# williamyang98/FM-Radio

Measured on AMD Instinct MI355X. Metric: IQ MSamples/sec demodulated to stereo+RDS per GPU; channels @ real-time, higher is better.
Workload: dtype f32 (tolerance mode: FIR operands split into 2 x bf16 on the matrix cores, 3 products per tap, fp32 accumulate; everything else fp32)

## Files before the change

### fm-radio_amd/capi.py

```python
from __future__ import annotations

import ctypes as C
import re
import subprocess
from pathlib import Path
from typing import NamedTuple

import numpy as np

PKG_DIR = Path(__file__).resolve().parent
ROOT = PKG_DIR.parent
CSRC = PKG_DIR / "csrc"
HEADER = ROOT / "include" / "fmdemod.h"
DEBUG_HEADER = ROOT / "include" / "fmdemod_debug.h"

FMD_AUDIO_LPR, FMD_AUDIO_LMR, FMD_AUDIO_STEREO = 0, 1, 2
FMD_FLAG_KEEP_TAPS = 1
FMD_FLAG_NO_PIPELINE = 2
FMD_FLAG_PLL_TIME_PARALLEL = 4
FMD_FLAG_PLL_LOW_WORK = 8
FMD_FLAG_PLL_K8 = 16
FMD_FLAG_PLL_STREAM_ORDER = 32
FMD_FLAG_FAST_MATH = 64
FMD_FLAG_RDS_DECODE = 128
# ... 325 lines not shown
    L.fmd_get_rds_symbols.argtypes = [H, C.c_void_p, C.c_void_p]
    L.fmd_get_rds_bytes.argtypes = [H, C.c_void_p, C.c_int, C.c_void_p]
    L.fmd_rds_bytes_dev.argtypes = [H, C.POINTER(C.c_void_p), C.POINTER(C.c_void_p), C.POINTER(C.c_int)]
    L.fmd_get_stream.argtypes = [H, C.c_char_p, C.c_void_p, C.c_size_t, C.POINTER(C.c_size_t)]
    L.fmd_selftest_atan2.argtypes = [C.c_void_p, C.c_void_p, C.c_void_p, C.c_size_t]
    L.fmd_selftest_atan2_table.argtypes = [C.c_void_p, C.c_void_p, C.c_void_p, C.c_size_t]
    L.fmd_selftest_atan2_table_u8.argtypes = [C.c_void_p, C.c_void_p, C.c_void_p, C.c_size_t]
    L.fmd_selftest_atan2_small.argtypes = [C.c_void_p, C.c_void_p, C.c_void_p, C.c_void_p, C.c_size_t]
    L.fmd_selftest_fast_math.argtypes = [C.c_int, C.c_void_p, C.c_void_p, C.c_void_p, C.c_size_t]
    L.fmd_get_spec_stats.argtypes = [H, C.c_void_p, C.c_int]
    L.fmd_design_pll_span.argtypes = [C.c_int, C.c_void_p, C.c_void_p, C.c_void_p, C.c_void_p]
    L.fmd_profile_enable.argtypes = [H, C.c_int]
    L.fmd_debug_split_front.argtypes = [H, C.c_int]
    L.fmd_debug_pll_adaptive.argtypes = [H, C.c_int, C.c_int]
    L.fmd_debug_extract_pairing.argtypes = [H, C.c_int]
    L.fmd_debug_plan.argtypes = [C.POINTER(Config), C.c_int, C.c_int, C.c_int, C.POINTER(PlanInfo)]
    L.fmd_debug_block_plan.argtypes = [C.POINTER(Config), C.POINTER(PlanFacts), C.c_int, C.POINTER(BlockPlanInfo)]
    L.fmd_profile_read.argtypes = [H, C.POINTER(KernelTime), C.c_int, C.POINTER(C.c_int)]
    L.fmd_chan_design.argtypes = [C.c_double, C.c_double, C.c_int, C.c_void_p, C.POINTER(C.c_int), C.POINTER(C.c_int)]
    L.fmd_chan_default_taps_per_phase.restype = C.c_int
    L.fmd_chan_default_taps_per_phase.argtypes = [C.c_double, C.c_double]
    L.fmd_chan_create.argtypes = [C.POINTER(ChanConfig), C.POINTER(C.c_void_p)]
    L.fmd_chan_reset.argtypes = [C.c_void_p]
    L.fmd_chan_info.argtypes = [C.c_void_p] + [C.POINTER(C.c_int)] * 4
    L.fmd_chan_get_taps.argtypes = [C.c_void_p, C.c_void_p, C.c_size_t]
    for fmt in ("cf32", "u8", "s8", "s16"):
        getattr(L, f"fmd_chan_process_{fmt}_dev").argtypes = [C.c_void_p, C.c_void_p, C.c_size_t, C.c_void_p, C.c_size_t, C.POINTER(C.c_size_t), C.c_void_p]
    L.fmd_scan_default_nfft.restype = C.c_int
    L.fmd_scan_default_nfft.argtypes = [C.c_double]
    L.fmd_scan_default_params.restype = None
# ... 471 lines not shown
        return rc

    def wait_input(self, stream=None):
        stream = _stream_ptr(stream)
        self._check(self.L.fmd_wait_input(self.h, C.c_void_p(stream)))

    def synchronize(self):
        self._check(self.L.fmd_synchronize(self.h))

    def pll_adaptive(self, k16_max_channels: int, time_parallel_max_channels: int = 7168) -> None:
        self._check(self.L.fmd_debug_pll_adaptive(self.h, int(k16_max_channels), int(time_parallel_max_channels)))

    def set_extract_pairing(self, mode: int) -> None:
        self._check(self.L.fmd_debug_extract_pairing(self.h, int(mode)))

    def set_output_lag(self, on: bool) -> None:
        self._check(self.L.fmd_set_output_lag(self.h, 1 if on else 0))

    def outputs_block(self) -> int:
        b = C.c_long(-1)
        self._check(self.L.fmd_outputs_block(self.h, C.byref(b)))
        return int(b.value)

    def wait_outputs(self, stream=None):
        stream = _stream_ptr(stream)
        self._check(self.L.fmd_wait_outputs(self.h, C.c_void_p(stream)))

    def release_outputs(self, stream=None):
        stream = _stream_ptr(stream)
        self._check(self.L.fmd_release_outputs(self.h, C.c_void_p(stream)))
# ... 1027 lines not shown
```

### fm-radio_amd/csrc/fmd_api.cpp

```cpp
#include <hip/hip_runtime.h>

#include <algorithm>
#include <cstdarg>
#include <cstdio>
#include <cstdlib>
#include <cstring>
#include <map>
#include <new>
#include <string>
#include <vector>

#include "fmd_design.h"
#include "fmd_kernels.h"
#include "fmd_plan.h"
#include "fmd_schedule.h"
#include "fmd_tables.h"
#include "fmdemod.h"
#include "fmdemod_debug.h"

using namespace fmd;

struct ProfiledBlock { hipEvent_t t0[ST_COUNT], t1[ST_COUNT]; bool used[ST_COUNT]; };

struct fmd_handle_s {
    fmd_config cfg{};
    LaunchCtx ctx{};
    fmd_coeffs base{};
    std::vector<fmd_controls> controls;
    bool controls_dirty = true;
    bool deemph_on = false;
    bool deemph_linger = false;
    std::vector<void*> allocs;
    void* d_in = nullptr;
// ... 467 lines not shown
    h->pipelined = (cfg->flags & FMD_FLAG_NO_PIPELINE) == 0;
    if (h->pipelined) warn_hw_queues_once();
    {
        std::vector<hipEvent_t*> evs = {&h->ev_in};
        for (int i = 0; i < kSlots; i++) { evs.push_back(&h->ev_P[i]); evs.push_back(&h->ev_F[i]); evs.push_back(&h->ev_A[i]); evs.push_back(&h->ev_B[i]); evs.push_back(&h->ev_E[i]); evs.push_back(&h->ev_X[i]); evs.push_back(&h->ev_C[i]); evs.push_back(&h->ev_D[i]); }
        for (hipEvent_t* ev : evs) {
            hipError_t e = hipEventCreateWithFlags(ev, hipEventDisableTiming);
            if (e != hipSuccess) return bail(fail(h, FMD_ERR_DEVICE, "event: %s", hipGetErrorString(e)));
        }
    }
    h->ctx.d = dims_of(*cfg, m);
    const Dims& d = h->ctx.d;
    h->ctx.plan = make_plan(d.C, d.m, d.n_fm_out, d.n_est, cfg->flags);
    refresh_block_plan(h->ctx);
    h->ctx.pll_unlocked_now = false; h->ctx.pll_launch_no = 0;
    h->bytes_cap = 16 * (d.n_rds / 256 + 1);
    h->ctx.bytes_cap = h->bytes_cap;
    h->ctx.keep_taps = (cfg->flags & FMD_FLAG_KEEP_TAPS) ? 1 : 0;
    h->ctx.rds_decode = (cfg->flags & FMD_FLAG_RDS_DECODE) ? 1 : 0;
    h->ctx.fast = (cfg->flags & FMD_FLAG_FAST_MATH) ? 1 : 0;

    fmd_controls def;
    fmd_default_controls(&def);
    h->controls.assign((size_t)d.C, def);
    design_all(&h->base, cfg->fs_baseband, &def);
    fill_ctx_coeffs(h);

    Buffers& b = h->ctx.b;
    const size_t C = (size_t)d.C;
    int rc = FMD_OK;
// ... 624 lines not shown
    *out = fmd_block_plan_info{b.iq_streams, (int)b.front, (int)in.front_input, in.front_tile, b.front_warmup, in.front_workgroups, b.front_lds_pad,
                               (int)in.predecim, in.predecim_tile, in.predecim_workgroups, b.deemph_pilot_sums, b.deemph_workgroups, p.power_rows,
                               (int)b.lmr_phase, b.extract_tile, b.extract_bp, b.extract_nt, b.extract_pair, b.extract_grid_x, (int)b.rds, b.rds_partials};
    return FMD_OK;
}

int fmd_debug_extract_pairing(fmd_handle h, int mode) {
    if (!h || mode < 0 || mode > 2) return FMD_ERR_ARG;
    int rc = fmd_synchronize(h);
    if (rc) return rc;
    h->ctx.facts.extract_pairing = mode;
    refresh_block_plan(h->ctx);
    return FMD_OK;
}

int fmd_profile_enable(fmd_handle h, int on) {
    if (!h) return FMD_ERR_ARG;
    h->sched.set_profiling(on < 0 ? 0 : (on > 3 ? 3 : on));
    return FMD_OK;
}

int fmd_profile_read(fmd_handle h, fmd_kernel_time* out, int cap, int* n_out) {
    if (!h || !out || !n_out || cap <= 0) return FMD_ERR_ARG;
    int rc = fmd_synchronize(h);
    if (rc) return rc;
    int n = 0;
    for (ProfiledBlock* pm : h->marks) {
        for (int i = 0; i < ST_COUNT; i++) {
            if (!pm->used[i]) continue;
            float ms = 0.0f;
// ... 187 lines not shown
```

### fm-radio_amd/csrc/fmd_kernels.h

```cpp
#pragma once

#include <hip/hip_runtime.h>
#include <stdint.h>
#include <cstdlib>

#include "fmd_plan.h"
#include "fmd_schedule.h"
#include "fmd_tables.h"
#include "fmdemod.h"

namespace fmd {

#ifdef FMD_DEV_HOOKS
inline const char* dev_env(const char* name) { return std::getenv(name); }
#else
inline const char* dev_env(const char*) { return nullptr; }
#endif

struct FrontTaps {
    float b_fm_in[64];
    float b_fm_out[64];
    float b_hilbert_odd[32];
    float fm_gain;
};
// ... 125 lines not shown
    Dims d;
    Buffers b;
    FrontTaps front;
    RdsTaps rds_taps;
    LoopCoeffs loops;
    int keep_taps;
    int fast;
    int bytes_cap;
    int rds_decode;
    RdsDecBufs rds_dec;
    Plan plan;
    PlanFacts facts;
    BlockPlan block;
    Dims d_front;
    unsigned pll_launch_no;
    bool pll_unlocked_now;
};

inline void refresh_block_plan(LaunchCtx& ctx) {
    ctx.block = make_block_plan(ctx.plan, ctx.facts);
    ctx.d_front = ctx.d;
    if (ctx.d.m > 1) { ctx.d_front.N = ctx.d.n_fm_in; ctx.d_front.m = 1; }
}

inline TapPtrs tap_ptrs(const LaunchCtx& ctx, int buf) {
    TapPtrs t{};
    float* p = ctx.b.taps[buf];
    if (!p) return t;
    const size_t nf = (size_t)ctx.d.C * ctx.d.n_fm_out, nr = (size_t)ctx.d.C * ctx.d.n_rds;
    t.pilot = reinterpret_cast<float2*>(p); p += 2 * nf;
// ... 31 lines not shown
```

### fm-radio_amd/csrc/fmd_kernels.hip

```cpp
#include "fmd_kernels.h"
#include <hip/hip_ext.h>
#include <cstdlib>
#include <type_traits>
#include "fmd_math.h"

#define FMD_LAUNCH(r, first, last, kern, grid, block, lds, s, ...)                                                   \
    do {                                                                                                             \
        hipEvent_t e0_ = (first) ? (r).t0 : nullptr, e1_ = (last) ? ((r).t1 ? (r).t1 : (r).done) : nullptr;         \
        if (e0_ || e1_) hipExtLaunchKernelGGL(kern, grid, block, lds, s, e0_, e1_, 0, __VA_ARGS__);                  \
        else hipLaunchKernelGGL(kern, grid, block, lds, s, __VA_ARGS__);                                             \
    } while (0)


namespace fmd {

static constexpr int kWave = 64;

__device__ __forceinline__ float& st(float* state, int field, int C, int c) { return state[(size_t)field * C + c]; }

#include "fmd_kernels_sparse.inc"

static constexpr int kDeemphWarmup = 128;
template <int TT = 512>
struct FrontGeom {
// ... 364 lines not shown
        }
    }
}

template <typename InT, int TT, int WU, bool FUSED = false>
__global__ __launch_bounds__(256, FUSED ? 6 : 5) void k_front_mfma(Dims d, const InT* __restrict__ in, const float2* __restrict__ tail_in,
                                                    float2* __restrict__ tail_out, float* __restrict__ fo_pl, float fm_gain,
                                                    const float* __restrict__ deemph, const uint4* __restrict__ tab, float4* __restrict__ pv_pl,
                                                    const PllSparseTab* __restrict__ sp, PllFusedArgs pf) {
    using G = FrontGeomM<TT, WU>;
    constexpr int T = G::T, NW = G::NW;
    extern __shared__ __attribute__((aligned(16))) float smem[];
    int bid = (int)blockIdx.x;
    if constexpr (FUSED) {
        if (bid < pf.n_wg) {
            pll_sparse_body(d, bid * 4 + (int)(threadIdx.x >> 6), (int)(threadIdx.x & (kWave - 1)), pf.pv, pf.hist_in, pf.hist_out, pf.fo, pf.fo_next, pf.poly, pf.poly_next,
                            pf.state, pf.k, pf.tab, 0, pf.spec_stats);
            return;
        }
        bid -= pf.n_wg;
    }
    float* theta = smem + G::OFF_THETA;

    const int tiles = d.n_fm_out / T;
    const int c = bid / tiles, tile = bid % tiles, o0 = tile * T, tid = threadIdx.x;
    __builtin_assume(tid >= 0 && tid < 256);
    const int lane = tid & (kWave - 1), lq = lane >> 4;
    const int g_lo = 2 * o0 - G::TAIL;
    const InT* in_c = in + (size_t)c * d.N;
    const float2* tail_c = tail_in + (size_t)c * d.tail_base + (d.tail_base - G::TAIL);

    FrontOps op;
// ... 327 lines not shown
    static constexpr int MINWG = (U8 && M == 4) ? 5 : 4;
    static_assert(NCOLS % NSUB == 0 && NBS % 8 == 0 && SEG * (CS - 1) + 32 * KS <= NBS && GF::NWB >= NPH + 1, "geometry");
};
template <int M, typename InT, bool FUSED>
__global__ __launch_bounds__(256, (FUSED ? FrontPreGeom<M, sizeof(InT) == 2>::MINWG : 4)) void k_front_pre_mfma(Dims d, const InT* __restrict__ in, const float2* __restrict__ pre_tail_in, float2* __restrict__ pre_tail_out,
                                                           const float2* __restrict__ tail_in, float2* __restrict__ tail_out, float* __restrict__ fo_pl, float fm_gain,
                                                           const uint4* __restrict__ tab_pre, const uint4* __restrict__ tab, float4* __restrict__ pv_pl,
                                                           const PllSparseTab* __restrict__ sp, PllFusedArgs pf) {
    constexpr bool U8 = sizeof(InT) == 2;
    using G = FrontPreGeom<M, U8>;
    constexpr int NBS = G::NBS, KS = G::KS, SEG = G::SEG, NH = G::NH, NWD = G::NWD, CS = G::CS;
    extern __shared__ __attribute__((aligned(16))) float smem[];
    int bid = (int)blockIdx.x;
    if constexpr (FUSED) {
        if (bid < pf.n_wg) {
            pll_sparse_body(d, bid * 4 + (int)(threadIdx.x >> 6), (int)(threadIdx.x & (kWave - 1)), pf.pv, pf.hist_in, pf.hist_out, pf.fo, pf.fo_next, pf.poly, pf.poly_next,
                            pf.state, pf.k, pf.tab, 0, pf.spec_stats);
            return;
        }
        bid -= pf.n_wg;
    }
    uint32_t* arr = reinterpret_cast<uint32_t*>(smem);
    float* region = smem + G::ARR_WORDS;
    const int tiles = d.n_fm_out / 1024;
    const int c = bid / tiles, tile = bid % tiles, o0 = tile * 1024, tid = threadIdx.x;
    __builtin_assume(tid >= 0 && tid < 256);
    const int lane = tid & (kWave - 1), wv = tid >> 6, lrow = lane & 15, lq = lane >> 4;
    const int g_first = M * (2 * o0 - 64) + M - 64 - G::SH;
    const InT* in_c = in + (size_t)c * d.N;
    const float2* ptail_c = pre_tail_in + (size_t)c * G::HIST;
    auto word_of = [](int pair) { return pair + 4 * (pair / (SEG / 2)); };

// ... 1709 lines not shown

__global__ void k_reset(Dims d, float* __restrict__ state) {
    const int c = blockIdx.x * blockDim.x + threadIdx.x;
    if (c >= d.C) return;
    for (int f = 0; f < S_NUM_FIELDS; f++) st(state, f, d.C, c) = 0.0f;
    st(state, S_AGC_PILOT_GAIN, d.C, c) = 0.1f;
    st(state, S_AGC_RDS_GAIN, d.C, c) = 0.1f;
}

template <int... Vs, typename F>
static bool with_constant(int v, F&& f) { return ((v == Vs ? (f(std::integral_constant<int, Vs>{}), true) : false) || ...); }
static hipError_t launched(bool found) { return found ? hipGetLastError() : hipErrorInvalidConfiguration; }

static_assert(kDeemphWarmup == kFrontDeemphWarmup && PredecimGeom<4>::TP == 512 && PredecimGeom<8>::TP == 512, "fmd_plan.cpp's geometry");

static PllFusedArgs fused_pilot_args(const LaunchCtx& ctx, const SlotRef* pll) {
    const Buffers& b = ctx.b;
    if (!pll) { PllFusedArgs none{}; none.state = b.state; return none; }
    const int nxt = (pll->buf + 1) % kSlots;
    return PllFusedArgs{(ctx.d.C + 31) / 32, b.pv_pl[pll->buf], b.pv_hist[pll->par], b.pv_hist[pll->par ^ 1], b.fo_pl[pll->buf], b.fo_pl[nxt],
                        b.pll_poly[pll->buf], b.pll_poly[nxt], b.state, ctx.loops, b.sparse_tab, b.spec_stats};
}

template <typename InT, typename F>
static bool with_front_tile(int tile, F&& f) {
    if constexpr (sizeof(InT) == 4) return with_constant<512, 1024>(tile, f);
    else return with_constant<512, 1024, 2048>(tile, f);
}

template <typename InT>
static hipError_t launch_front(const LaunchCtx& ctx, const BlockPlan::Input& in, SlotRef r, const InT* d_iq, hipStream_t s, const SlotRef* pll) {
    const BlockPlan& bp = ctx.block;
    const Buffers& b = ctx.b;
    const Dims& d = ctx.d_front;
    if (bp.front == FrontKernel::FrontMfma) {
        const PllFusedArgs pf = fused_pilot_args(ctx, pll);
        return launched(with_front_tile<InT>(in.front_tile, [&](auto tt) { with_constant<0, kDeemphWarmup>(bp.front_warmup, [&](auto wu) { with_constant<0, 1>(pll != nullptr, [&](auto fused) {
            constexpr int TT = decltype(tt)::value, WU = decltype(wu)::value;
            using G = FrontGeomM<TT, WU>;
            FMD_LAUNCH(r, true, true, (k_front_mfma<InT, TT, WU, decltype(fused)::value != 0>), dim3((unsigned)(in.front_workgroups + pf.n_wg)), dim3(256),
                       sizeof(float) * G::LDS_FLOATS + bp.front_lds_pad, s, d, d_iq, b.base_tail[r.par], b.base_tail[r.par ^ 1], b.fo_pl[r.buf], ctx.front.fm_gain,
                       b.deemph, b.front_mfma, b.pv_pl[r.buf], b.sparse_tab, pf);
        }); }); }));
    }
    return launched(with_front_tile<InT>(in.front_tile, [&](auto tt) {
        constexpr int TT = decltype(tt)::value;
        FMD_LAUNCH(r, true, true, (k_front<InT, TT>), dim3((unsigned)in.front_workgroups), dim3(256), sizeof(float) * FrontGeom<TT>::LDS_FLOATS, s, d, d_iq, b.base_tail[r.par],
                   b.base_tail[r.par ^ 1], b.fm_out_iq[r.buf], b.fm_out[r.buf], b.fo_tail[r.par ^ 1], ctx.front, ctx.facts.any_deemph ? 1 : 0);
    }));
}

template <int M, typename InT>
static void launch_front_pre(const LaunchCtx& ctx, const BlockPlan::Input& in, SlotRef r, const InT* d_iq, hipStream_t s, const SlotRef* pll) {
    using G = FrontPreGeom<M, sizeof(InT) == 2>;
    const Buffers& b = ctx.b;
    const PllFusedArgs pf = fused_pilot_args(ctx, pll);
    with_constant<0, 1>(pll != nullptr, [&](auto fused) {
        FMD_LAUNCH(r, true, true, (k_front_pre_mfma<M, InT, decltype(fused)::value != 0>), dim3((unsigned)(in.front_workgroups + pf.n_wg)), dim3(256), sizeof(float) * G::LDS_WORDS, s, ctx.d, d_iq,
                   b.pre_tail[r.par], b.pre_tail[r.par ^ 1], b.base_tail[r.par], b.base_tail[r.par ^ 1], b.fo_pl[r.buf], ctx.front.fm_gain, b.front_mfma + kFrontImgU4, b.front_mfma,
                   b.pv_pl[r.buf], b.sparse_tab, pf);
    });
}

template <int M, typename InT>
static void launch_predecim(const LaunchCtx& ctx, const BlockPlan::Input& in, SlotRef r, const InT* d_iq, hipStream_t s) {
    const Buffers& b = ctx.b;
    const dim3 grid((unsigned)in.predecim_workgroups);
    if (in.predecim == PredecimKernel::Mfma) {
        with_constant<256, (sizeof(InT) == 2 ? 8192 : 2048) / M>(in.predecim_tile, [&](auto tp) {
            FMD_LAUNCH(r, true, true, (k_predecim_mfma<M, InT, decltype(tp)::value>), grid, dim3(256), 0, s, ctx.d, d_iq, b.pre_tail[r.par], b.pre_tail[r.par ^ 1],
                       reinterpret_cast<float*>(b.fm_in[r.buf]), b.front_mfma + kFrontImgU4);
// ... 48 lines not shown
}

hipError_t launch_stage_power(const LaunchCtx& ctx, SlotRef r, hipStream_t s) {
    const Dims& d = ctx.d;
    return launched(with_constant<0, 1>(ctx.plan.power_rows, [&](auto rows) {
        FMD_LAUNCH(r, true, true, k_pilot_power<decltype(rows)::value != 0>, dim3(serial_waves(d)), dim3(kWave), 0, s, d, ctx.b.fm_out_iq[r.buf], ctx.b.pilot[r.buf], ctx.b.state,
                   ctx.loops, (int)S_PILOT_POWER0 + r.buf);
    }));
}

hipError_t launch_stage_pll(const LaunchCtx& ctx, SlotRef r, hipStream_t s) {
    const Dims& d = ctx.d;
    if (ctx.fast) {
        const int nxt = (r.buf + 1) % kSlots;
        const bool iq = ctx.block.iq_streams;
        FMD_LAUNCH(r, true, !iq && !r.warm, k_pll_sparse, dim3((unsigned)((d.C + 31) / 32)), dim3(4 * kWave), 0, s, d, ctx.b.pv_pl[r.buf], ctx.b.pv_hist[r.par], ctx.b.pv_hist[r.par ^ 1],
                   ctx.b.fo_pl[r.buf], ctx.b.fo_pl[nxt], ctx.b.pll_poly[r.buf], ctx.b.pll_poly[nxt], ctx.b.state, ctx.loops, ctx.b.sparse_tab, r.warm, ctx.b.spec_stats);
        if (r.warm)
            FMD_LAUNCH(r, false, !iq, k_pll_span, dim3((unsigned)((d.C + 3) / 4)), dim3(kWave), 0, s, d, ctx.b.fo_pl[r.buf], ctx.b.fo_pl[nxt],
                       ctx.b.pll_poly[r.buf], ctx.b.pll_poly[nxt], (float*)nullptr, ctx.b.state, ctx.loops, ctx.b.pilot_tab, ctx.b.span_tab, ctx.b.spec_stats, r.warm == 2 ? 1 : 0);
        if (iq) FMD_LAUNCH(r, false, false, k_poly_to_dt, dim3((unsigned)((size_t)d.n_fm_out * d.C / 256)), dim3(256), 0, s, d, ctx.b.pll_poly[r.buf], ctx.b.pll_dt[r.buf]);
        if (iq) FMD_LAUNCH(r, false, true, k_planes_to_iq, dim3((unsigned)(d.n_fm_out / 256 * d.C)), dim3(256), 0, s, d, ctx.b.fo_pl[r.buf], ctx.b.fm_out_iq[r.buf], ctx.front);
        return hipGetLastError();
    }
    if (ctx.b.taps[r.buf]) hipLaunchKernelGGL(k_pll_taps, dim3((unsigned)((d.C + kWave - 1) / kWave)), dim3(kWave), 0, s, d, ctx.b.pilot[r.buf], ctx.b.state, ctx.loops,
                                              (int)S_PILOT_POWER0 + r.buf, tap_ptrs(ctx, r.buf));
    const PllKernel kernel = pll_kernel(ctx.plan, ctx.pll_unlocked_now);
    if (kernel == PllKernel::LowWork) {
        FMD_LAUNCH(r, true, true, k_pilot_pll_pairs, dim3((unsigned)((d.C + kPllCh - 1) / kPllCh)), dim3(2 * kWave), 0, s, d, ctx.b.pilot[r.buf], ctx.b.pll_dt[r.buf],
                   ctx.b.state, ctx.loops, (int)S_PILOT_POWER0 + r.buf, ctx.b.spec_stats, ctx.b.pll_hint, ctx.pll_launch_no);
        return hipGetLastError();
    }
// ... 134 lines not shown
```

### fm-radio_amd/csrc/fmd_kernels_sparse.inc

```
static constexpr int kRowShr1 = 0x111, kRowShr2 = 0x112, kRowShr4 = 0x114, kRowShr8 = 0x118;
static constexpr int kWaveShr1 = 0x138, kRowBcast15 = 0x142;
template <int CTRL>
__device__ __forceinline__ float dpp_f(float old, float v, bool bound_zero) {
    return bound_zero ? __int_as_float(__builtin_amdgcn_update_dpp(0, __float_as_int(v), CTRL, 0xf, 0xf, true))
                      : __int_as_float(__builtin_amdgcn_update_dpp(__float_as_int(old), __float_as_int(v), CTRL, 0xf, 0xf, false));
}

struct __attribute__((packed, aligned(4))) F4U { float x, y, z, w; };
template <int CTRL, int BANK = 0xf>
__device__ __forceinline__ float dpp0(float v) {
    return __int_as_float(__builtin_amdgcn_update_dpp(0, __float_as_int(v), CTRL, 0xf, BANK, true));
}
__device__ __forceinline__ float sum8_all(float v) {
    v += dpp0<0xB1>(v);
    v += dpp0<0x4E>(v);
    v += dpp0<0x141>(v);
    return v;
}
__device__ __forceinline__ float bcast_lane7_of_8(float v) {
    const int q = __builtin_amdgcn_update_dpp(0, __float_as_int(v), 0xFF, 0xf, 0xf, true);
    return __int_as_float(__builtin_amdgcn_update_dpp(q, q, 0x104, 0xf, 0x5, false));
}
__device__ __forceinline__ float bcast_lane0_of_8(float v) {
    const int q = __builtin_amdgcn_update_dpp(0, __float_as_int(v), 0x00, 0xf, 0xf, true);
// ... 150 lines not shown
        }
    }
    if (spec_stats) {
        if (lane == 0) atomicAdd(&spec_stats[0], (unsigned long long)chunks);
        if (live && mine && kp == 0) { atomicAdd(&spec_stats[3], (unsigned long long)chunks); atomicAdd(&spec_stats[4], (unsigned long long)n); }
        if (lane == 0 && wave_id == 0) { atomicAdd(&spec_stats[6], __builtin_readcyclecounter() - clk0); atomicAdd(&spec_stats[7], __builtin_amdgcn_s_memrealtime() - rt0); }
    }
    if (live && kp < 4) hist_out[(size_t)cs * 4 + kp] = pvr[ncol - 4 + kp];
    if (live) {
        const float4* src = reinterpret_cast<const float4*>(fo + (size_t)cs * fo_stride + n);
        float4* dst = reinterpret_cast<float4*>(fo_next + (size_t)cs * fo_stride);
        for (int i = kp; i < kFoPad / 4; i += KP) dst[i] = src[i];
    }
}

__global__ __launch_bounds__(4 * kWave) void k_pll_sparse(Dims d, const float4* __restrict__ pv, const float4* __restrict__ hist_in, float4* __restrict__ hist_out,
                                                      const float* __restrict__ fo, float* __restrict__ fo_next,
                                                      float4* __restrict__ poly, float4* __restrict__ poly_next,
                                                      float* __restrict__ state, LoopCoeffs k, const PllSparseTab* __restrict__ tab, int warm_block,
                                                      unsigned long long* __restrict__ spec_stats) {
    pll_sparse_body(d, (int)(blockIdx.x * 4 + (threadIdx.x >> 6)), (int)(threadIdx.x & (kWave - 1)), pv, hist_in, hist_out, fo, fo_next, poly, poly_next, state, k, tab,
                    warm_block, spec_stats);
}

struct PllFusedArgs {
    int n_wg;
    const float4* pv; const float4* hist_in; float4* hist_out; const float* fo; float* fo_next; float4* poly; float4* poly_next; float* state; LoopCoeffs k; const PllSparseTab* tab; unsigned long long* spec_stats;
};

__global__ __launch_bounds__(256) void k_pilot_sums(Dims d, const float* __restrict__ fo_pl, float4* __restrict__ pv_pl, const PllSparseTab* __restrict__ sp) {
    const int n = d.n_fm_out, ncol = n / kSparseDec, blocks_per = (ncol + 63) / 64;
    const int c = blockIdx.x / blocks_per, cc = (blockIdx.x % blocks_per) * 64 + (threadIdx.x >> 2), part = threadIdx.x & 3;
    if (cc >= ncol) return;
    const float* x = fo_pl + (size_t)c * (kFoPad + n) + kFoPad + kSparseDec * cc;
    const float* w = ((part & 1) ? sp->wim : sp->wre) + ((part < 2) ? kSparseDec : 0);
    float a0_ = 0.0f, a1_ = 0.0f;
#pragma unroll
    for (int i = 0; i < kSparseDec; i += 2) { a0_ = fmaf(w[i], x[i], a0_); a1_ = fmaf(w[i + 1], x[i + 1], a1_); }
    reinterpret_cast<float*>(pv_pl + (size_t)c * ncol + cc)[part] = a0_ + a1_;
}

__global__ __launch_bounds__(256) void k_poly_to_dt(Dims d, const float4* __restrict__ poly, float* __restrict__ pll_dt) {
    const int n = d.n_fm_out, spans = n / kSpan;
// ... 9 lines not shown
```

Before: 275,000.

## Add rider PLL body packing 16 stations per wave for fused pilot stage

Adds a new sparse-PLL body in which each wave handles S stations instead of 8. Lanes compute span-phase points grouped eight per station and hand them through LDS to per-station loop-update lanes. The fused front-kernel pilot stage uses this body by default whenever enough LDS is available and the indices fit in 32 bits, which cuts the number of pilot workgroups. A debug switch selects the old body or the standalone rider kernel. The trade is extra LDS traffic and serialized per-chunk loop updates per lane in exchange for better lane utilization.

```diff
diff --git a/fm-radio_amd/capi.py b/fm-radio_amd/capi.py
--- a/fm-radio_amd/capi.py
+++ b/fm-radio_amd/capi.py
@@ -363,6 +363,7 @@
     L.fmd_debug_split_front.argtypes = [H, C.c_int]
     L.fmd_debug_pll_adaptive.argtypes = [H, C.c_int, C.c_int]
     L.fmd_debug_extract_pairing.argtypes = [H, C.c_int]
+    L.fmd_debug_pilot_body.argtypes = [H, C.c_int]
     L.fmd_debug_plan.argtypes = [C.POINTER(Config), C.c_int, C.c_int, C.c_int, C.POINTER(PlanInfo)]
     L.fmd_debug_block_plan.argtypes = [C.POINTER(Config), C.POINTER(PlanFacts), C.c_int, C.POINTER(BlockPlanInfo)]
     L.fmd_profile_read.argtypes = [H, C.POINTER(KernelTime), C.c_int, C.POINTER(C.c_int)]
@@ -864,6 +865,9 @@
     def set_extract_pairing(self, mode: int) -> None:
         self._check(self.L.fmd_debug_extract_pairing(self.h, int(mode)))
 
+    def set_pilot_body(self, mode: int) -> None:
+        self._check(self.L.fmd_debug_pilot_body(self.h, int(mode)))
+
     def set_output_lag(self, on: bool) -> None:
         self._check(self.L.fmd_set_output_lag(self.h, 1 if on else 0))
 
diff --git a/fm-radio_amd/csrc/fmd_api.cpp b/fm-radio_amd/csrc/fmd_api.cpp
--- a/fm-radio_amd/csrc/fmd_api.cpp
+++ b/fm-radio_amd/csrc/fmd_api.cpp
@@ -17,6 +17,7 @@
 #include "fmd_tables.h"
 #include "fmdemod.h"
 #include "fmdemod_debug.h"
+#include "fmdemod_pilot_debug.h"
 
 using namespace fmd;
 
@@ -514,6 +515,7 @@
     h->ctx.plan = make_plan(d.C, d.m, d.n_fm_out, d.n_est, cfg->flags);
     refresh_block_plan(h->ctx);
     h->ctx.pll_unlocked_now = false; h->ctx.pll_launch_no = 0;
+    h->ctx.pilot_body = 0;
     h->bytes_cap = 16 * (d.n_rds / 256 + 1);
     h->ctx.bytes_cap = h->bytes_cap;
     h->ctx.keep_taps = (cfg->flags & FMD_FLAG_KEEP_TAPS) ? 1 : 0;
@@ -1168,6 +1170,14 @@
     return FMD_OK;
 }
 
+int fmd_debug_pilot_body(fmd_handle h, int mode) {
+    if (!h || mode < 0 || mode > 2) return FMD_ERR_ARG;
+    int rc = fmd_synchronize(h);
+    if (rc) return rc;
+    h->ctx.pilot_body = mode;
+    return FMD_OK;
+}
+
 int fmd_profile_enable(fmd_handle h, int on) {
     if (!h) return FMD_ERR_ARG;
     h->sched.set_profiling(on < 0 ? 0 : (on > 3 ? 3 : on));
diff --git a/fm-radio_amd/csrc/fmd_kernels.h b/fm-radio_amd/csrc/fmd_kernels.h
--- a/fm-radio_amd/csrc/fmd_kernels.h
+++ b/fm-radio_amd/csrc/fmd_kernels.h
@@ -163,6 +163,7 @@
     BlockPlan block;
     Dims d_front;
     unsigned pll_launch_no;
+    int pilot_body;
     bool pll_unlocked_now;
 };
 
diff --git a/fm-radio_amd/csrc/fmd_kernels.hip b/fm-radio_amd/csrc/fmd_kernels.hip
--- a/fm-radio_amd/csrc/fmd_kernels.hip
+++ b/fm-radio_amd/csrc/fmd_kernels.hip
@@ -402,8 +402,7 @@
     int bid = (int)blockIdx.x;
     if constexpr (FUSED) {
         if (bid < pf.n_wg) {
-            pll_sparse_body(d, bid * 4 + (int)(threadIdx.x >> 6), (int)(threadIdx.x & (kWave - 1)), pf.pv, pf.hist_in, pf.hist_out, pf.fo, pf.fo_next, pf.poly, pf.poly_next,
-                            pf.state, pf.k, pf.tab, 0, pf.spec_stats);
+            fused_pilot_stage(d, bid, pf, smem);
             return;
         }
         bid -= pf.n_wg;
@@ -761,8 +760,7 @@
     int bid = (int)blockIdx.x;
     if constexpr (FUSED) {
         if (bid < pf.n_wg) {
-            pll_sparse_body(d, bid * 4 + (int)(threadIdx.x >> 6), (int)(threadIdx.x & (kWave - 1)), pf.pv, pf.hist_in, pf.hist_out, pf.fo, pf.fo_next, pf.poly, pf.poly_next,
-                            pf.state, pf.k, pf.tab, 0, pf.spec_stats);
+            fused_pilot_stage(d, bid, pf, smem);
             return;
         }
         bid -= pf.n_wg;
@@ -2502,11 +2500,13 @@
 
 static_assert(kDeemphWarmup == kFrontDeemphWarmup && PredecimGeom<4>::TP == 512 && PredecimGeom<8>::TP == 512, "fmd_plan.cpp's geometry");
 
-static PllFusedArgs fused_pilot_args(const LaunchCtx& ctx, const SlotRef* pll) {
+static PllFusedArgs fused_pilot_args(const LaunchCtx& ctx, const SlotRef* pll, size_t lds_bytes) {
     const Buffers& b = ctx.b;
     if (!pll) { PllFusedArgs none{}; none.state = b.state; return none; }
     const int nxt = (pll->buf + 1) % kSlots;
-    return PllFusedArgs{(ctx.d.C + 31) / 32, b.pv_pl[pll->buf], b.pv_hist[pll->par], b.pv_hist[pll->par ^ 1], b.fo_pl[pll->buf], b.fo_pl[nxt],
+    const bool rider = ctx.pilot_body != 1 && lds_bytes >= sizeof(float) * kRiderLdsFloats && rider_indexable(ctx.d);
+    const int per_wg = rider ? 4 * kRiderS : 32;
+    return PllFusedArgs{(ctx.d.C + per_wg - 1) / per_wg, rider ? 1 : 0, b.pv_pl[pll->buf], b.pv_hist[pll->par], b.pv_hist[pll->par ^ 1], b.fo_pl[pll->buf], b.fo_pl[nxt],
                         b.pll_poly[pll->buf], b.pll_poly[nxt], b.state, ctx.loops, b.sparse_tab, b.spec_stats};
 }
 
@@ -2522,10 +2522,10 @@
     const Buffers& b = ctx.b;
     const Dims& d = ctx.d_front;
     if (bp.front == FrontKernel::FrontMfma) {
-        const PllFusedArgs pf = fused_pilot_args(ctx, pll);
         return launched(with_front_tile<InT>(in.front_tile, [&](auto tt) { with_constant<0, kDeemphWarmup>(bp.front_warmup, [&](auto wu) { with_constant<0, 1>(pll != nullptr, [&](auto fused) {
             constexpr int TT = decltype(tt)::value, WU = decltype(wu)::value;
             using G = FrontGeomM<TT, WU>;
+            const PllFusedArgs pf = fused_pilot_args(ctx, pll, sizeof(float) * G::LDS_FLOATS + bp.front_lds_pad);
             FMD_LAUNCH(r, true, true, (k_front_mfma<InT, TT, WU, decltype(fused)::value != 0>), dim3((unsigned)(in.front_workgroups + pf.n_wg)), dim3(256),
                        sizeof(float) * G::LDS_FLOATS + bp.front_lds_pad, s, d, d_iq, b.base_tail[r.par], b.base_tail[r.par ^ 1], b.fo_pl[r.buf], ctx.front.fm_gain,
                        b.deemph, b.front_mfma, b.pv_pl[r.buf], b.sparse_tab, pf);
@@ -2542,7 +2542,7 @@
 static void launch_front_pre(const LaunchCtx& ctx, const BlockPlan::Input& in, SlotRef r, const InT* d_iq, hipStream_t s, const SlotRef* pll) {
     using G = FrontPreGeom<M, sizeof(InT) == 2>;
     const Buffers& b = ctx.b;
-    const PllFusedArgs pf = fused_pilot_args(ctx, pll);
+    const PllFusedArgs pf = fused_pilot_args(ctx, pll, sizeof(float) * G::LDS_WORDS);
     with_constant<0, 1>(pll != nullptr, [&](auto fused) {
         FMD_LAUNCH(r, true, true, (k_front_pre_mfma<M, InT, decltype(fused)::value != 0>), dim3((unsigned)(in.front_workgroups + pf.n_wg)), dim3(256), sizeof(float) * G::LDS_WORDS, s, ctx.d, d_iq,
                    b.pre_tail[r.par], b.pre_tail[r.par ^ 1], b.base_tail[r.par], b.base_tail[r.par ^ 1], b.fo_pl[r.buf], ctx.front.fm_gain, b.front_mfma + kFrontImgU4, b.front_mfma,
@@ -2621,8 +2621,12 @@
     if (ctx.fast) {
         const int nxt = (r.buf + 1) % kSlots;
         const bool iq = ctx.block.iq_streams;
-        FMD_LAUNCH(r, true, !iq && !r.warm, k_pll_sparse, dim3((unsigned)((d.C + 31) / 32)), dim3(4 * kWave), 0, s, d, ctx.b.pv_pl[r.buf], ctx.b.pv_hist[r.par], ctx.b.pv_hist[r.par ^ 1],
-                   ctx.b.fo_pl[r.buf], ctx.b.fo_pl[nxt], ctx.b.pll_poly[r.buf], ctx.b.pll_poly[nxt], ctx.b.state, ctx.loops, ctx.b.sparse_tab, r.warm, ctx.b.spec_stats);
+        if (ctx.pilot_body == 2 && rider_indexable(d))
+            FMD_LAUNCH(r, true, !iq && !r.warm, k_pll_sparse_rider, dim3((unsigned)((d.C + 4 * kRiderS - 1) / (4 * kRiderS))), dim3(4 * kWave), 0, s, d, ctx.b.pv_pl[r.buf], ctx.b.pv_hist[r.par],
+                       ctx.b.pv_hist[r.par ^ 1], ctx.b.fo_pl[r.buf], ctx.b.fo_pl[nxt], ctx.b.pll_poly[r.buf], ctx.b.pll_poly[nxt], ctx.b.state, ctx.loops, ctx.b.sparse_tab, r.warm, ctx.b.spec_stats);
+        else
+            FMD_LAUNCH(r, true, !iq && !r.warm, k_pll_sparse, dim3((unsigned)((d.C + 31) / 32)), dim3(4 * kWave), 0, s, d, ctx.b.pv_pl[r.buf], ctx.b.pv_hist[r.par], ctx.b.pv_hist[r.par ^ 1],
+                       ctx.b.fo_pl[r.buf], ctx.b.fo_pl[nxt], ctx.b.pll_poly[r.buf], ctx.b.pll_poly[nxt], ctx.b.state, ctx.loops, ctx.b.sparse_tab, r.warm, ctx.b.spec_stats);
         if (r.warm)
             FMD_LAUNCH(r, false, !iq, k_pll_span, dim3((unsigned)((d.C + 3) / 4)), dim3(kWave), 0, s, d, ctx.b.fo_pl[r.buf], ctx.b.fo_pl[nxt],
                        ctx.b.pll_poly[r.buf], ctx.b.pll_poly[nxt], (float*)nullptr, ctx.b.state, ctx.loops, ctx.b.pilot_tab, ctx.b.span_tab, ctx.b.spec_stats, r.warm == 2 ? 1 : 0);
diff --git a/fm-radio_amd/csrc/fmd_kernels_sparse.inc b/fm-radio_amd/csrc/fmd_kernels_sparse.inc
--- a/fm-radio_amd/csrc/fmd_kernels_sparse.inc
+++ b/fm-radio_amd/csrc/fmd_kernels_sparse.inc
@@ -188,6 +188,213 @@
     }
 }
 
+template <int S>
+__device__ __forceinline__ void pll_rider_body(const Dims& d, int wave_id, int lane, const float4* __restrict__ pv, const float4* __restrict__ hist_in,
+                                               float4* __restrict__ hist_out, const float* __restrict__ fo, float* __restrict__ fo_next,
+                                               float4* __restrict__ poly, float4* __restrict__ poly_next,
+                                               float* __restrict__ state, const LoopCoeffs& k, const PllSparseTab* __restrict__ tab,
+                                               int warm_block, unsigned long long* __restrict__ spec_stats, float* __restrict__ lds) {
+    constexpr int KP = kSparsePts, D = kSparseDec, CH = kSpan;
+    constexpr int NG = S / 8;
+    constexpr int U = 2;
+    constexpr int SZ = S * KP;
+    static_assert(KP == 8 && D == 16 && (S == 16 || S == 32 || S == 64), "lane = one of 8 points of a span in zpart, lane = station in the loop update");
+    const unsigned long long clk0 = __builtin_readcyclecounter(), rt0 = __builtin_amdgcn_s_memrealtime();
+    const int g = lane >> 3, kp = lane & 7;
+    const int n = d.n_fm_out, chunks = n / CH, ncol = n / D;
+    const size_t fo_stride = (size_t)kFoPad + n, po_stride = (size_t)1 + chunks;
+    auto group_station = [&](int j) __attribute__((always_inline)) { const int c = wave_id * S + 8 * j + g; return c < d.C ? c : d.C - 1; };
+    auto group_live = [&](int j) __attribute__((always_inline)) { return wave_id * S + 8 * j + g < d.C; };
+    const int sl = lane & (S - 1), c = wave_id * S + sl;
+    const bool live = lane < S && c < d.C;
+    const int cs = c < d.C ? c : d.C - 1;
+
+    const float rot_r = tab->rot[kp][0], rot_i = tab->rot[kp][1];
+    const float cy_r = tab->carry[kp][0], cy_i = tab->carry[kp][1];
+    auto uni = [](float v) __attribute__((always_inline)) { return __int_as_float(__builtin_amdgcn_readfirstlane(__float_as_int(v))); };
+    const float s1r = uni(tab->scan[0][0]), s1i = uni(tab->scan[0][1]), s2r = uni(tab->scan[1][0]), s2i = uni(tab->scan[1][1]), s4r = uni(tab->scan[2][0]), s4i = uni(tab->scan[2][1]);
+    const float phi0 = uni(tab->phi0), inv_s2 = uni(tab->inv_s2), nbar = uni(tab->nbar), kappa = uni(tab->kappa), k2r = uni(tab->kap2[0]), k2i = uni(tab->kap2[1]);
+    const float b0 = uni(k.pll_b0), b1 = uni(k.pll_b1), a0 = uni(k.pll_a0);
+    const float Ts = 1.0f / 128000.0f, ktsi = 0.1f * Ts;
+    const float two_pi = bits_f32(kTwoPiBits);
+    float ckk[KP], nk1k[KP];
+#pragma unroll
+    for (int i = 0; i < KP; i++) { ckk[i] = uni(tab->ck[i]); nk1k[i] = uni(tab->nk1[i]); }
+    float rw[kSpanRows][7];
+#pragma unroll
+    for (int r = 0; r < kSpanRows; r++) {
+        rw[r][0] = uni(tab->wsum[r]); rw[r][1] = uni(tab->wmom[r]);
+#pragma unroll
+        for (int i = 0; i < 5; i++) rw[r][2 + i] = uni(tab->s[r][i]);
+    }
+
+    float Zr[NG], Zi[NG], power[NG];
+#pragma unroll
+    for (int j = 0; j < NG; j++) { Zr[j] = st(state, SA_X1R, d.C, group_station(j)); Zi[j] = st(state, SA_X2R, d.C, group_station(j)); power[j] = 0.0f; }
+    float lpf = st(state, S_PLL_Y1, d.C, cs), integ = st(state, S_PLL_INT, d.C, cs);
+    float e1 = st(state, S_PLL_ERR, d.C, cs), e2 = st(state, S_PLL_X1, d.C, cs), tprev = st(state, S_PLL_T, d.C, cs);
+    const bool mine = !(warm_block && (warm_block == 2 || st(state, SA_X1I, d.C, cs) < kPllWarmSamples));
+
+    struct Pt { float2 nw, od; };
+    auto fetch0 = [&](int j) __attribute__((always_inline)) {
+        const float4* pvr = pv + (size_t)group_station(j) * ncol;
+        const float4* hst = hist_in + (size_t)group_station(j) * 4 + 4;
+        const int cn = kp - 2, co = cn - 1;
+        const float4* pn = cn < 0 ? hst + cn : pvr + cn;
+        const float4* po = co < 0 ? hst + co : pvr + co;
+        return Pt{reinterpret_cast<const float2*>(pn)[0], reinterpret_cast<const float2*>(po)[1]};
+    };
+    unsigned col0[NG];
+#pragma unroll
+    for (int j = 0; j < NG; j++) col0[j] = (unsigned)group_station(j) * (unsigned)ncol + (unsigned)(kp - 2);
+    auto fetch = [&](int j, int q) __attribute__((always_inline)) {
+        const unsigned cn = col0[j] + (unsigned)((q < chunks ? q : chunks - 1) * KP);
+        const char* pn = reinterpret_cast<const char*>(pv) + (size_t)(cn * 16u);
+        return Pt{*reinterpret_cast<const float2*>(pn), *reinterpret_cast<const float2*>(pn - 8)};
+    };
+    auto zpart = [&](const Pt& xq, float& Zr_, float& Zi_, float& power_) __attribute__((always_inline)) {
+        const float ur = xq.nw.x + xq.od.x, ui = xq.nw.y + xq.od.y;
+        float vr = fmaf(rot_r, ur, -(rot_i * ui)), vi = fmaf(rot_r, ui, rot_i * ur);
+        const float v0r = vr, v0i = vi;
+        {
+            float tr = dpp0<kRowShr1>(vr), ti = dpp0<kRowShr1>(vi);
+            tr = (kp >= 1) ? tr : 0.0f; ti = (kp >= 1) ? ti : 0.0f;
+            vr = fmaf(s1r, tr, fmaf(-s1i, ti, vr)); vi = fmaf(s1r, ti, fmaf(s1i, tr, vi));
+            tr = dpp0<kRowShr2>(vr); ti = dpp0<kRowShr2>(vi);
+            tr = (kp >= 2) ? tr : 0.0f; ti = (kp >= 2) ? ti : 0.0f;
+            vr = fmaf(s2r, tr, fmaf(-s2i, ti, vr)); vi = fmaf(s2r, ti, fmaf(s2i, tr, vi));
+            tr = dpp0<kRowShr4, 0xA>(vr); ti = dpp0<kRowShr4, 0xA>(vi);
+            vr = fmaf(s4r, tr, fmaf(-s4i, ti, vr)); vi = fmaf(s4r, ti, fmaf(s4i, tr, vi));
+        }
+        const float zr = fmaf(cy_r, Zr_, fmaf(-cy_i, Zi_, vr)), zi = fmaf(cy_r, Zi_, fmaf(cy_i, Zr_, vi));
+        Zr_ = bcast_lane7_of_8(zr); Zi_ = bcast_lane7_of_8(zi);
+        power_ += fmaf(zr, zr, zi * zi);
+        return fast_atan2_turns(fmaf(k2r, v0i, fmaf(k2i, v0r, zi)), fmaf(k2r, v0r, fmaf(-k2i, v0i, zr))) + phi0;
+    };
+    auto tree8 = [](const float (&v)[KP]) __attribute__((always_inline)) { return ((v[0] + v[1]) + (v[2] + v[3])) + ((v[7] + v[6]) + (v[5] + v[4])); };
+
+    Pt nx[NG];
+#pragma unroll
+    for (int j = 0; j < NG; j++) nx[j] = fetch0(j);
+#pragma unroll
+    for (int j = 0; j < NG; j++) {
+        lds[j * kWave + lane] = zpart(nx[j], Zr[j], Zi[j], power[j]);
+        nx[j] = fetch(j, 1);
+    }
+    for (int q0 = 0; q0 < chunks; q0 += U) {
+#pragma unroll
+      for (int jq = 0; jq < U; jq++) {
+        const int q = q0 + jq;
+        if (jq + 1 < U || q + 1 < chunks) {
+#pragma unroll
+            for (int j = 0; j < NG; j++) {
+                lds[((jq + 1) & 1) * SZ + j * kWave + lane] = zpart(nx[j], Zr[j], Zi[j], power[j]);
+                nx[j] = fetch(j, q + 2);
+                __builtin_amdgcn_sched_barrier(0);
+            }
+        }
+        __builtin_amdgcn_wave_barrier();
+        const float4 pa = *reinterpret_cast<const float4*>(lds + (jq & 1) * SZ + sl * KP), pb = *reinterpret_cast<const float4*>(lds + (jq & 1) * SZ + sl * KP + 4);
+        __builtin_amdgcn_wave_barrier();
+        const float phi[KP] = {pa.x, pa.y, pa.z, pa.w, pb.x, pb.y, pb.z, pb.w};
+        const float lpf0 = fmaf(b0, e2, fmaf(b1, e1, a0 * lpf));
+        const float ig0 = clampf(fmaf(ktsi, e1, integ), -1.0f, 1.0f);
+        const float u0 = fmaf(lpf0, 0.01f, ig0);
+        const float cc = clampf(u0, -1.0f, 1.0f);
+        const float F0 = fmaf(cc, -100.0f, -19000.0f);
+        const float gq = F0 + 19000.0f;
+        const float r0 = fmaf(100.0f, cc, gq);
+        const float dq = fmaf(gq, Ts, kappa);
+        const float tb = tprev;
+        float ek[KP], wk[KP];
+#pragma unroll
+        for (int i = 0; i < KP; i++) { ek[i] = fmaf(nk1k[i], dq, phi[i] + tb); ek[i] = ek[i] - rintf(ek[i]); }
+        const float ek0 = ek[0];
+#pragma unroll
+        for (int i = 0; i < KP; i++) { const float dk = ek[i] - ek0; ek[i] = ek0 + (dk - rintf(dk)); wk[i] = ckk[i] * ek[i]; }
+        const float am = tree8(ek) * 0.125f, bs = tree8(wk) * inv_s2;
+        float rowv[kSpanRows];
+#pragma unroll
+        for (int r = 0; r < kSpanRows; r++) {
+            const float sv = fmaf(rw[r][2], lpf, fmaf(rw[r][3], integ, fmaf(rw[r][4], e1, fmaf(rw[r][5], e2, rw[r][6] * r0))));
+            rowv[r] = fmaf(rw[r][0], am, fmaf(rw[r][1], bs, sv));
+        }
+        const float f0 = fmaf(-nbar, bs, am), f127 = fmaf(127.0f - nbar, bs, am);
+        float e_last = f127, e_prev = f127 - bs;
+        if (__builtin_amdgcn_ballot_w64(fabsf(f0) >= 0.5f || fabsf(f127) >= 0.5f) != 0ull) {
+            const float r_lo = rintf(f0), r_hi = rintf(f127);
+            if (r_lo != 0.0f || r_hi != 0.0f) {
+                int ns = 0;
+                if (r_hi != r_lo) {
+                    const float edge = (r_hi > r_lo) ? r_hi - 0.5f : r_hi + 0.5f;
+                    const float xs = ceilf((edge - f0) / bs);
+                    ns = (int)fminf(fmaxf(xs, 0.0f), (float)kSpan);
+                }
+#pragma unroll
+                for (int r = 0; r < kSpanRows; r++) rowv[r] -= fmaf(r_hi - r_lo, tab->sw[r][ns], r_lo * tab->sw[r][0]);
+            }
+        }
+        const float u_end = fmaf(rowv[0], 0.01f, clampf(rowv[1], -1.0f, 1.0f));
+        const bool railed = fabsf(u0) >= 1.0f && fabsf(u_end) >= 1.0f && u0 * u_end > 0.0f;
+        const float al = railed ? 0.0f : rowv[2], be = railed ? 0.0f : rowv[3], ga = railed ? 0.0f : rowv[4];
+        const float d3 = fmaf(fmaf(fmaf(ga, (float)(CH - 1), be), (float)(CH - 1), al), (float)(CH - 1), 0.0f);
+        const float4 pc = make_float4(tb + dq, dq + al, be, ga);
+        if (live && mine) {
+            poly[(size_t)cs * po_stride + 1 + q] = pc;
+            if (q == chunks - 1) poly_next[(size_t)cs * po_stride] = pc;
+        }
+        lpf = rowv[0];
+        integ = clampf(rowv[1], -1.0f, 1.0f);
+        const float g_end = -100.0f * fmaf(lpf, 0.01f, integ);
+        const float d3m = d3 - Ts * (g_end - gq);
+        float en = e_last + d3, ep = e_prev + d3m;
+        en = en - rintf(en); ep = ep - rintf(ep);
+        e1 = en * two_pi; e2 = ep * two_pi;
+        float tn = fmaf((float)CH, dq, tb) + d3;
+        tprev = tn - rintf(tn);
+      }
+    }
+#pragma unroll
+    for (int j = 0; j < NG; j++) {
+        const float pw = sum8_all(power[j]) * tab->pw_scale;
+        const int cj = group_station(j);
+        if (group_live(j) && kp == 0) {
+            st(state, SA_X1R, d.C, cj) = Zr[j]; st(state, SA_X2R, d.C, cj) = Zi[j];
+            if (!(warm_block && (warm_block == 2 || st(state, SA_X1I, d.C, cj) < kPllWarmSamples))) {
+                float gain = st(state, S_AGC_PILOT_GAIN, d.C, cj);
+                const float target_gain = sqrtf((1.0f / pw) * (float)n);
+                gain = fmaf(target_gain - gain, 0.2f, gain);
+                st(state, S_AGC_PILOT_GAIN, d.C, cj) = gain;
+            }
+        }
+    }
+    if (live && mine) {
+        st(state, S_PLL_Y1, d.C, c) = lpf; st(state, S_PLL_INT, d.C, c) = integ;
+        st(state, S_PLL_ERR, d.C, c) = e1; st(state, S_PLL_X1, d.C, c) = e2; st(state, S_PLL_T, d.C, c) = tprev;
+    }
+    if (spec_stats) {
+        if (lane == 0) atomicAdd(&spec_stats[0], (unsigned long long)chunks * NG);
+        if (live && mine) { atomicAdd(&spec_stats[3], (unsigned long long)chunks); atomicAdd(&spec_stats[4], (unsigned long long)n); }
+        if (lane == 0 && wave_id == 0) { atomicAdd(&spec_stats[6], __builtin_readcyclecounter() - clk0); atomicAdd(&spec_stats[7], __builtin_amdgcn_s_memrealtime() - rt0); }
+    }
+#pragma unroll
+    for (int j = 0; j < NG; j++) {
+        if (!group_live(j)) continue;
+        const int cj = group_station(j);
+        if (kp < 4) hist_out[(size_t)cj * 4 + kp] = pv[(size_t)cj * ncol + ncol - 4 + kp];
+        const float4* src = reinterpret_cast<const float4*>(fo + (size_t)cj * fo_stride + n);
+        float4* dst = reinterpret_cast<float4*>(fo_next + (size_t)cj * fo_stride);
+        for (int i = kp; i < kFoPad / 4; i += KP) dst[i] = src[i];
+    }
+}
+
+#ifndef FMD_PILOT_RIDER_S
+#define FMD_PILOT_RIDER_S 16
+#endif
+static constexpr int kRiderS = FMD_PILOT_RIDER_S;
+static constexpr int kRiderLdsFloats = 4 * 2 * kRiderS * kSparsePts;
+__host__ __device__ inline bool rider_indexable(const Dims& d) { return (unsigned long long)d.C * (unsigned long long)(d.n_fm_out / kSparseDec) * 16ull < (1ull << 32); }
+
 __global__ __launch_bounds__(4 * kWave) void k_pll_sparse(Dims d, const float4* __restrict__ pv, const float4* __restrict__ hist_in, float4* __restrict__ hist_out,
                                                       const float* __restrict__ fo, float* __restrict__ fo_next,
                                                       float4* __restrict__ poly, float4* __restrict__ poly_next,
@@ -197,10 +404,31 @@
                     warm_block, spec_stats);
 }
 
+__global__ __launch_bounds__(4 * kWave) void k_pll_sparse_rider(Dims d, const float4* __restrict__ pv, const float4* __restrict__ hist_in, float4* __restrict__ hist_out,
+                                                            const float* __restrict__ fo, float* __restrict__ fo_next,
+                                                            float4* __restrict__ poly, float4* __restrict__ poly_next,
+                                                            float* __restrict__ state, LoopCoeffs k, const PllSparseTab* __restrict__ tab, int warm_block,
+                                                            unsigned long long* __restrict__ spec_stats) {
+    __shared__ __attribute__((aligned(16))) float phases[kRiderLdsFloats];
+    const int wv = (int)(threadIdx.x >> 6);
+    pll_rider_body<kRiderS>(d, (int)(blockIdx.x * 4) + wv, (int)(threadIdx.x & (kWave - 1)), pv, hist_in, hist_out, fo, fo_next, poly, poly_next, state, k, tab,
+                            warm_block, spec_stats, phases + wv * (kRiderLdsFloats / 4));
+}
+
 struct PllFusedArgs {
     int n_wg;
+    int rider;
     const float4* pv; const float4* hist_in; float4* hist_out; const float* fo; float* fo_next; float4* poly; float4* poly_next; float* state; LoopCoeffs k; const PllSparseTab* tab; unsigned long long* spec_stats;
 };
+
+__device__ __forceinline__ void fused_pilot_stage(const Dims& d, int bid, const PllFusedArgs& pf, float* __restrict__ smem) {
+    const int wv = (int)(threadIdx.x >> 6), lane = (int)(threadIdx.x & (kWave - 1));
+    if (pf.rider)
+        pll_rider_body<kRiderS>(d, bid * 4 + wv, lane, pf.pv, pf.hist_in, pf.hist_out, pf.fo, pf.fo_next, pf.poly, pf.poly_next, pf.state, pf.k, pf.tab, 0, pf.spec_stats,
+                                smem + wv * (kRiderLdsFloats / 4));
+    else
+        pll_sparse_body(d, bid * 4 + wv, lane, pf.pv, pf.hist_in, pf.hist_out, pf.fo, pf.fo_next, pf.poly, pf.poly_next, pf.state, pf.k, pf.tab, 0, pf.spec_stats);
+}
 
 __global__ __launch_bounds__(256) void k_pilot_sums(Dims d, const float* __restrict__ fo_pl, float4* __restrict__ pv_pl, const PllSparseTab* __restrict__ sp) {
     const int n = d.n_fm_out, ncol = n / kSparseDec, blocks_per = (ncol + 63) / 64;
diff --git a/include/fmdemod_pilot_debug.h b/include/fmdemod_pilot_debug.h
--- /dev/null
+++ b/include/fmdemod_pilot_debug.h
@@ -0,0 +1,15 @@
+#ifndef FMDEMOD_PILOT_DEBUG_H
+#define FMDEMOD_PILOT_DEBUG_H
+
+#include "fmdemod.h"
+
+#ifdef __cplusplus
+extern "C" {
+#endif
+
+int fmd_debug_pilot_body(fmd_handle h, int mode);
+
+#ifdef __cplusplus
+}
+#endif
+#endif
```

Result: slower. 269,100 (-2.1%).
